# filippo-orru/path-tracer-rust

Measured on AMD Instinct MI355X. Metric: ray_bounces_per_sec, higher is better.
Workload: dtype f32

## Files before the change

### path-tracer-rust_amd/csrc/pt_kernels.hip

```cpp
#include <cstdio>
#include <cstdlib>
#include <string>

#include "pt_kernels.h"
#ifdef PT_TU_TILE
#include "pt_tile.h"
#endif

namespace pt {

#ifdef PT_TU_TILE
typedef TileParams MegaParams;
#define k_mega k_tile_mega
#define k_mega_cand k_tile_mega_cand
#else
typedef FrameParams MegaParams;
#endif
#if defined(PT_TU_FLAT) || defined(PT_TU_TILE)
#define PT_TU_PART 1
#endif

void set_error(const std::string &m);

extern __shared__ uint4 dyn_lds[];

constexpr uint32_t kCandDeferFlush = 64;

__device__ __forceinline__ uint32_t rfl(uint32_t v) { return (uint32_t)__builtin_amdgcn_readfirstlane((int)v); }
__device__ __forceinline__ uint32_t lane_prefix(uint64_t mask) {
    return __builtin_amdgcn_mbcnt_hi((uint32_t)(mask >> 32), __builtin_amdgcn_mbcnt_lo((uint32_t)mask, 0u));
}

struct StreamSlice {
    char *base;
    uint32_t off_tp, off_od1;
};
__device__ __forceinline__ StreamSlice slice_of(const RayQueue &q, uint32_t b, uint32_t cap) {
    StreamSlice s;
    s.base = q.buf + (size_t)b * cap * kRayBytes;
    s.off_tp = cap * 16u;
    s.off_od1 = cap * 32u;
    return s;
}
__device__ __forceinline__ float4 ld_od0(const StreamSlice &q, uint32_t i) { return *reinterpret_cast<const float4 *>(q.base + i * 16u); }
__device__ __forceinline__ float4 ld_tp(const StreamSlice &q, uint32_t i) { return *reinterpret_cast<const float4 *>(q.base + (i * 16u + q.off_tp)); }
__device__ __forceinline__ float2 ld_od1(const StreamSlice &q, uint32_t i) { return *reinterpret_cast<const float2 *>(q.base + (i * 8u + q.off_od1)); }
__device__ __forceinline__ void store_ray(const StreamSlice &q, uint32_t slot, vec3 o, vec3 d, vec3 thr, uint32_t word) {
    *reinterpret_cast<float4 *>(q.base + slot * 16u) = make_float4(o.x, o.y, o.z, d.x);
    *reinterpret_cast<float2 *>(q.base + (slot * 8u + q.off_od1)) = make_float2(d.y, d.z);
    *reinterpret_cast<float4 *>(q.base + (slot * 16u + q.off_tp)) = make_float4(thr.x, thr.y, thr.z, __uint_as_float(word));
}
__device__ __forceinline__ void load_ray_slice(const StreamSlice &q, uint32_t i, vec3 &o, vec3 &d, vec3 &thr, uint32_t &word) {
    const float4 a = ld_od0(q, i);
    const float4 tp = ld_tp(q, i);
    const float2 c = ld_od1(q, i);
    o = mk(a.x, a.y, a.z);
    d = mk(a.w, c.x, c.y);
    thr = mk(tp.x, tp.y, tp.z);
    word = __float_as_uint(tp.w);
}
__device__ __forceinline__ void load_ray_slice(const StreamSlice &q, uint32_t i, RayRows &ray, f32x4 &tp) {
    const f32x2 *a = reinterpret_cast<const f32x2 *>(q.base + i * 16u);
    ray.p0 = a[0];
    ray.p1 = a[1];
    tp = *reinterpret_cast<const f32x4 *>(q.base + (i * 16u + q.off_tp));
    ray.p2 = *reinterpret_cast<const f32x2 *>(q.base + (i * 8u + q.off_od1));
}

#ifndef PT_TU_PART
template <bool PROBE>
__global__ __launch_bounds__(kBlock) void k_generate(FrameParams F, RayQueue q, uint32_t *__restrict__ cnt0,
                                                     uint32_t cap, uint32_t s0, uint32_t s_here, uint32_t m) {
    const uint32_t b = blockIdx.x, tid = threadIdx.x;
    const StreamSlice qs = slice_of(q, b, cap);
    const uint32_t mb = stream_pixel_count(F.npix, F.n_streams, b);
    const uint32_t n = mb * s_here;
    for (uint32_t g = tid; g < n; g += kBlock) {
        const uint32_t pl = stream_pixel(F.n_streams, b, g % mb);
        const uint32_t s = s0 + g / mb;
        const PathRay r = primary_ray<PROBE>(F, global_pixel(F, pl), s);
        store_ray(qs, g, r.o, r.d, r.thr, pack_word(g % mb, g / mb, PROBE ? F.depth0 : 0u, 1u));
    }
    if (tid == 0) cnt0[b] = n;
}

constexpr uint32_t kParkCap = 128;
__host__ __device__ inline size_t bvh_park_offset(const DevScene &S, uint32_t block) {
    return (bvh_lds_bytes(S, block) + 15) & ~(size_t)15;
}
__host__ __device__ inline size_t bvh_park_bytes(uint32_t block) { return (size_t)(block / 64u) * kParkCap * 36u; }

template <bool BVH>
__global__ __launch_bounds__(BVH ? kBlockBvh : kBlock, BVH ? 5 : 1) void k_intersect(DevScene S, RayQueue q, float2 *__restrict__ hit,
                                                      const uint32_t *__restrict__ cnt, uint32_t cap,
                                                      unsigned long long *__restrict__ blk_rays) {
    const uint32_t b = blockIdx.x, tid = threadIdx.x;
    const uint32_t n = cnt[b];
    const size_t base = (size_t)b * cap;
    const StreamSlice qs = slice_of(q, b, cap);
    if (!BVH) {
        for (uint32_t i = tid; i < n; i += blockDim.x) {
            const float4 a = ld_od0(qs, i);
            const float2 c = ld_od1(qs, i);
            const HitRec h = intersect_scene_dev<false>(S, mk(a.x, a.y, a.z), mk(a.w, c.x, c.y), dyn_lds);
            hit[base + i] = make_float2(h.t, __int_as_float(h.id));
        }
    } else {
        if (n != 0u) stage_bvh(S, dyn_lds);
        char *park = reinterpret_cast<char *>(dyn_lds) + bvh_park_offset(S, blockDim.x) + (size_t)(tid >> 6) * kParkCap * 36u;
        float4 *const pa = reinterpret_cast<float4 *>(park), *const pb = pa + kParkCap;
        uint32_t *const pi = reinterpret_cast<uint32_t *>(pb + kParkCap);
        const uint32_t lane = tid & 63u;
        uint32_t n_park = 0;
        auto walk = [&](uint32_t e, bool valid) {
            if (valid) {
                const float4 a = pa[e], bq = pb[e];
                const uint32_t idx = pi[e];
                const vec3 o = mk(a.x, a.y, a.z), d = mk(a.w, bq.x, bq.y);
                float best_t = bq.z;
                int32_t best_id = __float_as_int(bq.w);
                if (walk_deferred(S, o, d, dyn_lds, best_t, best_id)) {
                    const HitRec h = scan_scene<true, true>(S, o, d, dyn_lds);
                    best_t = h.t;
                    best_id = h.id;
                }
                hit[base + idx] = make_float2(best_t, __int_as_float(best_id));
            }
        };
        for (uint32_t j0 = 0; j0 < n; j0 += blockDim.x) {
            const uint32_t i = j0 + tid;
            bool want = false;
            vec3 o = mk(0, 0, 0), d = o;
            HitRec h;
            h.t = 0.0f;
            h.id = -1;
            if (i < n) {
                const float4 a = ld_od0(qs, i);
                const float2 c = ld_od1(qs, i);
                o = mk(a.x, a.y, a.z);
                d = mk(a.w, c.x, c.y);
                h = intersect_scene_dev<true, true>(S, o, d, dyn_lds, &want);
                if (!want) hit[base + i] = make_float2(h.t, __int_as_float(h.id));
            }
            const uint64_t mw = __builtin_amdgcn_ballot_w64(want);
            if (mw != 0ull) {
                if (want) {
                    const uint32_t e = n_park + lane_prefix(mw);
                    pa[e] = make_float4(o.x, o.y, o.z, d.x);
                    pb[e] = make_float4(d.y, d.z, h.t, __int_as_float(h.id));
                    pi[e] = i;
                }
                n_park += (uint32_t)__builtin_popcountll(mw);
            }
            if (n_park >= 64u) {
                n_park -= 64u;
                walk(n_park + lane, true);
            }
        }
        if (n_park != 0u) walk(lane, lane < n_park);
    }
    if (tid == 0) blk_rays[b] += n;
}

#endif

template <bool STAGED>
__global__ __launch_bounds__(kBlock, PT_ISECT_WAVES) void k_intersect_cand(DevScene S, RayQueue q, float2 *__restrict__ hit,
                                                              const uint32_t *__restrict__ cnt, uint32_t cap,
                                                              unsigned long long *__restrict__ blk_rays) {
    const uint32_t b = blockIdx.x, tid = threadIdx.x, lane = tid & 63u;
    const uint32_t n = cnt[b];
    if (n == 0u) return;
    CandLds cand;
    {
        char *wbase = reinterpret_cast<char *>(dyn_lds) + (size_t)(tid >> 6) * kCandWaveBytes;
        cand.ray_a = reinterpret_cast<float4 *>(wbase);
        cand.keys = reinterpret_cast<unsigned long long *>(wbase + 128u * 16u);
        cand.ray_b = reinterpret_cast<float2 *>(wbase + 128u * 24u);
        cand.queue = reinterpret_cast<uint16_t *>(wbase + 128u * 32u);
        char *sbase = reinterpret_cast<char *>(dyn_lds) + intersect_cand_lds_bytes();
        cand.staged = reinterpret_cast<const CandPairRec *>(sbase);
        cand.surf = S.surf;
        if (STAGED) {
            const uint4 *src = reinterpret_cast<const uint4 *>(S.cand_pairs);
            uint4 *dst = reinterpret_cast<uint4 *>(sbase);
            const uint32_t n_rows = S.n_cand_pairs * (uint32_t)(sizeof(CandPairRec) / 16u);
            for (uint32_t k = tid; k < n_rows; k += kBlock) dst[k] = src[k];
            __syncthreads();
        }
    }
    const StreamSlice qin = slice_of(q, b, cap);
    float2 *const hit_b = hit + (size_t)b * cap;
    CandRing ring;
    ring.head = 0u;
    ring.count = 0u;
    const uint32_t n_chunks = (n + kBlock - 1u) / kBlock;
    bool prev_valid = false;
#if PT_ISECT_PREFETCH
    float4 na = make_float4(0.0f, 0.0f, 0.0f, 0.0f);
    float2 nc = make_float2(0.0f, 0.0f);
    if (tid < n) {
        na = ld_od0(qin, tid);
        nc = ld_od1(qin, tid);
    }
#endif
    for (uint32_t it = 0; it <= n_chunks; ++it) {
        const uint32_t par = it & 1u;
        const uint32_t i = it * kBlock + tid;
        const bool cur_valid = it < n_chunks && i < n;
        const uint32_t pending = ring.count;
        bool ran_batch = false;
        if (it < n_chunks) {
            vec3 o = mk(0.0f, 0.0f, 0.0f), d = o;
#if PT_ISECT_PREFETCH
            if (cur_valid) {
                o = mk(na.x, na.y, na.z);
                d = mk(na.w, nc.x, nc.y);
            }
// ... 173 lines not shown
    float4 *const dbuf = reinterpret_cast<float4 *>(reinterpret_cast<char *>(dyn_lds) + pass_lds_defer_offset(m)) +
                         (size_t)(tid >> 6) * (3u * kDeferCap);
    uint32_t n_defer = 0;
    StreamSlice qout{};
    uint32_t *tail_p = nullptr;
    auto append = [&](const ShadeOut &so, uint32_t word) {
        const uint64_t m1 = __builtin_amdgcn_ballot_w64(so.n_rays >= 1);
        const uint64_t m2 = __builtin_amdgcn_ballot_w64(so.n_rays == 2);
        const uint32_t c1 = (uint32_t)__builtin_popcountll(m1), c2 = (uint32_t)__builtin_popcountll(m2);
        if ((c1 + c2) == 0u) return;
        uint32_t wbase = 0;
        if ((tid & 63u) == 0u) wbase = atomicAdd(tail_p, c1 + c2);
        wbase = (uint32_t)__builtin_amdgcn_readfirstlane((int)wbase);
        if (so.n_rays >= 1) {
            const uint32_t slot = wbase + lane_prefix(m1);
            if (slot < cap)
                store_ray(qout, slot, so.x, so.d0, so.thr0,
                          pack_word(word_pix(word), word_sample(word), meta_depth(so.meta0), meta_branch(so.meta0)));
            else
                overflow = true;
        }
        if (so.n_rays == 2) {
            const uint32_t slot = wbase + c1 + lane_prefix(m2);
            if (slot < cap)
                store_ray(qout, slot, so.x, so.d1, so.thr1,
                          pack_word(word_pix(word), word_sample(word), meta_depth(so.meta1), meta_branch(so.meta1)));
            else
                overflow = true;
        }
    };
    auto shade_deferred = [&](uint32_t e, bool valid) {
        ShadeOut so;
        so.n_rays = 0;
        so.emits = false;
        uint32_t word = 0;
        if (valid) {
            const float4 a = dbuf[e], bq = dbuf[kDeferCap + e], cq = dbuf[2u * kDeferCap + e];
            PathRay in;
            in.o = mk(a.x, a.y, a.z);
            in.d = mk(a.w, bq.x, bq.y);
            in.thr = mk(bq.z, bq.w, cq.x);
            word = __float_as_uint(cq.y);
            HitRec h;
            h.t = cq.z;
            h.id = __float_as_int(cq.w);
            in.pix = lds_pix[word_pix(word)];
            in.meta = pack_meta(s0 + word_sample(word), word_depth(word), word_branch(word));
            shade_hit<kShadeRefractOnly>(S, P, in, h, so);
            if (so.emits) add_radiance_lds(lds_acc, m, word_pix(word), so.contrib);
        }
        append(so, word);
    };
    for (uint32_t depth = 0; depth < (uint32_t)kMaxDepth && n != 0u; ++depth) {
        const StreamSlice qin = slice_of((depth & 1u) ? q1 : q0, b, cap);
        qout = slice_of((depth & 1u) ? q0 : q1, b, cap);
        __syncthreads();
        if (tid == 0) s_tail_p[(depth + 1u) & 1u] = 0u;
        tail_p = s_tail_p + (depth & 1u);
        total += n;
        for (uint32_t j0 = 0; j0 < n; j0 += kBlock) {
            const uint32_t i = j0 + tid;
            PathRay in;
            uint32_t word = 0;
            if (i < n) {
                if (depth == 0u) {
                    const uint32_t pj = i % mb, sj = i / mb;
                    in = primary_ray<PROBE>(F, lds_pix[pj], s0 + sj);
                    word = pack_word(pj, sj, PROBE ? F.depth0 : 0u, 1u);
                } else {
                    const float4 a = ld_od0(qin, i);
                    const float4 tp = ld_tp(qin, i);
                    const float2 c = ld_od1(qin, i);
                    in.o = mk(a.x, a.y, a.z);
                    in.d = mk(a.w, c.x, c.y);
                    in.thr = mk(tp.x, tp.y, tp.z);
                    word = __float_as_uint(tp.w);
                }
            }
            ShadeOut so;
            so.n_rays = 0;
            so.emits = false;
            so.deferred = false;
            HitRec h;
            h.t = 0.0f;
            h.id = -1;
            if (i < n) {
                h = intersect_scene_dev<false>(S, in.o, in.d, nullptr);
                if (h.id >= 0) {
                    in.pix = lds_pix[word_pix(word)];
                    in.meta = pack_meta(s0 + word_sample(word), word_depth(word), word_branch(word));
                    shade_hit<DEFER ? kShadeDeferRefract : kShadeAll>(S, P, in, h, so);
                    if (so.emits) add_radiance_lds(lds_acc, m, word_pix(word), so.contrib);
                }
            }
            append(so, word);
            const uint64_t md = DEFER ? __builtin_amdgcn_ballot_w64(so.deferred) : 0ull;
            if (DEFER && md != 0ull) {
                if (so.deferred) {
                    const uint32_t e = n_defer + lane_prefix(md);
                    dbuf[e] = make_float4(in.o.x, in.o.y, in.o.z, in.d.x);
                    dbuf[kDeferCap + e] = make_float4(in.d.y, in.d.z, in.thr.x, in.thr.y);
                    dbuf[2u * kDeferCap + e] = make_float4(in.thr.z, __uint_as_float(word), h.t, __int_as_float(h.id));
                }
                n_defer = rfl(n_defer + (uint32_t)__builtin_popcountll(md));
            }
            if (DEFER && n_defer >= 64u) {
                n_defer -= 64u;
                shade_deferred(n_defer + (tid & 63u), true);
            }
        }
        if (DEFER && n_defer != 0u) {
            shade_deferred(tid & 63u, (tid & 63u) < n_defer);
            n_defer = 0u;
        }
        __syncthreads();
        const uint32_t tail = *tail_p;
        n = tail < cap ? tail : cap;
    }
    if (overflow) atomicOr(flags, 1u);
    __syncthreads();
    if (tid == 0) blk_rays[b] += total;
    const size_t plane = (size_t)F.n_streams * m;
    for (uint32_t k = tid; k < 3u * mb; k += kBlock) {
        const uint32_t c = k / mb, p = k - c * mb;
        const unsigned long long v = lds_acc[c * m + p];
        if (v) acc[(size_t)c * plane + (size_t)b * m + p] += v;
    }
}

#endif
constexpr uint32_t kCandParkCap = kWaveParkCap;

template <bool STAGED, bool DEFER, bool BVH, bool PROBE, bool NLDS = false>
__global__ __launch_bounds__(kBlock, BVH ? PT_CAND_BVH_WAVES : PT_CAND_WAVES) void k_pass_cand(DevScene S, FrameParams F, RayQueue q0, RayQueue q1, uint32_t cap,
                                                         uint32_t s0, uint32_t s_here, uint32_t m,
                                                         unsigned long long *__restrict__ acc,
                                                         unsigned long long *__restrict__ blk_rays,
                                                         uint32_t *__restrict__ flags) {
    unsigned long long *lds_acc = reinterpret_cast<unsigned long long *>(dyn_lds);
    uint32_t *s_tail_p = reinterpret_cast<uint32_t *>(lds_acc + pass_acc_slots(m));
    const uint32_t b = blockIdx.x, tid = threadIdx.x, lane = tid & 63u;
    const uint32_t mb = stream_pixel_count(F.npix, F.n_streams, b);
    if (mb == 0u) return;
#ifdef PT_PHASE_STATS
    unsigned long long ph_t0, ph_r0;
    phase_begin(&ph_t0, &ph_r0);
#endif
    for (uint32_t k = tid; k < 3u * m; k += kBlock) lds_acc[k] = 0ull;
    if (tid == 0) s_tail_p[0] = s_tail_p[1] = 0u;
    if (tid == 0) {
        float *cw = reinterpret_cast<float *>(s_tail_p + 4);
        cw[0] = F.lens_x, cw[1] = F.lens_y, cw[2] = F.lens_z, cw[3] = F.cam_px, cw[4] = F.cam_py, cw[5] = F.cam_pz;
        cw[6] = F.su_x, cw[7] = F.su_y, cw[8] = F.su_z, cw[9] = F.sv_x, cw[10] = F.sv_y, cw[11] = F.sv_z;
        s_tail_p[16] = F.width, s_tail_p[17] = F.height;
    }
    uint32_t *lds_pix = s_tail_p + kPassTailWords;
    uint32_t *lds_px = lds_pix + m, *lds_py = lds_px + m;
    for (uint32_t j = tid; j < mb; j += kBlock) {
        const uint32_t pix = global_pixel(F, stream_pixel(F.n_streams, b, j));
        lds_pix[j] = pix;
        lds_px[j] = pix % F.width;
        lds_py[j] = F.height - 1u - pix / F.width;
    }
    const uint32_t wv = (uint32_t)__builtin_amdgcn_readfirstlane((int)(tid >> 6));
    const uint32_t cap_w = cap >> 2;
    const uint32_t n0 = mb * s_here;
    const uint32_t n_chunks = (n0 + 63u) >> 6;
    const uint32_t my_chunks = (n_chunks + 3u - wv) >> 2;
    const uint32_t quarter = (((n_chunks + 3u) >> 2) << 6) < n0 ? (((n_chunks + 3u) >> 2) << 6) : n0;
    const uint32_t base0 = wv << 6;
    uint32_t gen_left = 0u;
    if (my_chunks != 0u) {
        const uint32_t last = wv + ((my_chunks - 1u) << 2);
        gen_left = ((my_chunks - 1u) << 6) + (n0 - (last << 6) < 64u ? n0 - (last << 6) : 64u);
    }
#if PT_SAMPLE_MAJOR
    const uint32_t step_q = 256u / s_here, step_r = 256u % s_here;
    uint32_t gen_pj = (base0 + lane) / s_here, gen_sj = (base0 + lane) % s_here;
#else
    const uint32_t step_q = 256u / mb, step_r = 256u % mb;
    uint32_t gen_pj = (base0 + lane) % mb, gen_sj = (base0 + lane) / mb;
#endif
    CandLds cand;
    const SurfRec *surf_lds = nullptr;
    uint32_t surf_head = 0u;
    {
        char *cbase = reinterpret_cast<char *>(dyn_lds) + pass_lds_cand_offset(m, DEFER);
        char *wbase = cbase + (size_t)(tid >> 6) * kCandWaveBytes;
        cand.ray_a = reinterpret_cast<float4 *>(wbase);
        cand.keys = reinterpret_cast<unsigned long long *>(wbase + 128u * 16u);
        cand.ray_b = reinterpret_cast<float2 *>(wbase + 128u * 24u);
        cand.queue = reinterpret_cast<uint16_t *>(wbase + 128u * 32u);
        char *sbase = cbase + pass_lds_cand_bytes() + (BVH ? pass_cand_bvh_bytes(S) : 0u);
        cand.staged = reinterpret_cast<const CandPairRec *>(sbase);
        cand.surf = S.surf;
        if (STAGED) {
            const uint4 *src = reinterpret_cast<const uint4 *>(S.cand_pairs);
            uint4 *dst = reinterpret_cast<uint4 *>(sbase);
            const uint32_t n_rows = S.n_cand_pairs * (uint32_t)(sizeof(CandPairRec) / 16u);
            for (uint32_t k = tid; k < n_rows; k += kBlock) dst[k] = src[k];
            if (!BVH || S.surf_staged) {
                const uint4 *src2 = reinterpret_cast<const uint4 *>(S.surf);
                uint4 *dst2 = dst + n_rows;
                const uint32_t n_rows2 = (S.n_objs + S.n_tris) * (uint32_t)(sizeof(SurfRec) / 16u);
                for (uint32_t k = tid; k < n_rows2; k += kBlock) dst2[k] = src2[k];
                cand.surf = reinterpret_cast<const SurfRec *>(dst2);
            } else if (S.surf_head != 0u) {
                const uint4 *src2 = reinterpret_cast<const uint4 *>(S.surf);
                uint4 *dst2 = dst + n_rows;
                const uint32_t n_rows2 = S.surf_head * (uint32_t)(sizeof(SurfRec) / 16u);
                for (uint32_t k = tid; k < n_rows2; k += kBlock) dst2[k] = src2[k];
                surf_lds = reinterpret_cast<const SurfRec *>(dst2);
                surf_head = S.surf_head;
            }
        }
    }
    char *const walk_lds = (reinterpret_cast<char *>(dyn_lds) + pass_lds_cand_offset(m, DEFER) + pass_lds_cand_bytes());
    unsigned long long *p_key = nullptr;
    unsigned long long *walk_keys = nullptr;
    WalkQueue wq{};
    const WalkNode *const nodes_lds = reinterpret_cast<const WalkNode *>(walk_lds + pass_cand_nodes_offset(S));
    if (BVH && NLDS) {
        const uint4 *src = reinterpret_cast<const uint4 *>(walk_nodes(S));
        uint4 *dst = reinterpret_cast<uint4 *>(walk_lds + pass_cand_nodes_offset(S));
        for (uint32_t k = tid; k < walk_node_count(S) * (uint32_t)(sizeof(WalkNode) / 16u); k += kBlock) dst[k] = src[k];
    }
    if (BVH) {
        walk_keys = reinterpret_cast<unsigned long long *>(walk_lds + pass_cand_queues_bytes(S) + (size_t)(tid >> 6) * kCandWalkKeyBytes);
        char *qb = walk_lds + (size_t)(tid >> 6) * pass_cand_queue_bytes(S);
        wq.redo = reinterpret_cast<uint32_t *>(qb);
        wq.ent = reinterpret_cast<uint2 *>(qb + kWalkQueueHeader);
        wq.cap = (uint32_t)((pass_cand_queue_bytes(S) - kWalkQueueHeader) / 8u);
        if (S.walk_queue_cap >= 128u && S.walk_queue_cap < wq.cap) wq.cap = S.walk_queue_cap;
    }
    ShadeParams P;
    P.idx_begin = F.idx_begin;
    P.npix = F.npix;
    P.n_streams = F.n_streams;
    {
        uint32_t k_lo = F.seed_lo, k_hi = F.seed_hi;
        asm volatile("" : "+s"(k_lo), "+s"(k_hi));
        P.seed_lo = k_lo;
        P.seed_hi = k_hi;
    }
    P.debug = F.debug;
    P.s0 = s0;
    P.chunk_pixels = F.chunk_pixels;
    P.chunk_first = F.chunk_first;
    P.chunk_step = F.chunk_step;
    P.k_begin = F.k_begin;
    bool overflow = false;
    unsigned long long total = 0ull;
    const uint32_t room = cap_w < kWaveStackMax ? cap_w : kWaveStackMax;
    const bool room_for_all = 4u * quarter + 3u <= room;
    StreamSlice qs;
    qs.base = q0.buf + (size_t)(b * 4u + wv) * cap_w * kRayBytes;
    qs.off_tp = room * 16u;
    qs.off_od1 = room * 32u;
    StreamSlice qpark{};
    if (BVH || DEFER) {
        qpark.base = q1.buf + (size_t)(b * 4u + wv) * kWaveParkBytes;
        qpark.off_tp = kCandParkCap * 16u;
        qpark.off_od1 = kCandParkCap * 32u;
        p_key = reinterpret_cast<unsigned long long *>(qpark.base + kCandParkCap * kRayBytes);
    }
    if (!room_for_all && room < 512u) {
        if (tid == 0) atomicOr(flags, 2u);
        return;
    }
    uint32_t top = 0u;
    auto append = [&](const ShadeOut &so, uint32_t word) {
        PT_PHASE(kPhAppend);
        const uint64_t m1 = __builtin_amdgcn_ballot_w64(so.n_rays >= 1);
        const uint64_t m2 = __builtin_amdgcn_ballot_w64(so.n_rays == 2);
        const uint32_t c1 = (uint32_t)__builtin_popcountll(m1), c2 = (uint32_t)__builtin_popcountll(m2);
        if ((c1 + c2) == 0u) return;
        const uint32_t wbase = top;
        if (wbase + c1 + c2 > room) {
            overflow = true;
            return;
        }
        top = rfl(top + c1 + c2);
        if (so.n_rays >= 1)
            store_ray(qs, wbase + lane_prefix(m1), so.x, so.d0, so.thr0,
                      pack_word(word_pix(word), word_sample(word), meta_depth(so.meta0), meta_branch(so.meta0)));
        if (so.n_rays == 2) {
            PT_PHASE(kPhAppend2);
            store_ray(qs, wbase + c1 + lane_prefix(m2), so.x, so.d1, so.thr1,
                      pack_word(word_pix(word), word_sample(word), meta_depth(so.meta1), meta_branch(so.meta1)));
        }
    };
    uint32_t n_defer = 0;
    auto shade_deferred = [&](uint32_t e, bool valid) {
        ShadeOut so;
        so.n_rays = 0;
        so.emits = false;
        uint32_t word = 0;
        PT_PHASE(kPhDefer);
        __builtin_amdgcn_fence(__ATOMIC_RELEASE, "wavefront");
        __builtin_amdgcn_fence(__ATOMIC_ACQUIRE, "wavefront");
        if (valid) {
            PathRay in;
            load_ray_slice(qpark, e, in.o, in.d, in.thr, word);
            const unsigned long long hk = p_key[e];
            in.pix = lds_pix[word_pix(word)];
            in.meta = pack_meta(s0 + word_sample(word), word_depth(word), word_branch(word));
            const Surface sf = fetch_surface_rank(cand.surf, in.o, in.d, __uint_as_float((uint32_t)(hk >> 32)), (uint32_t)hk);
            shade_surface<kShadeRefractOnly>(P, in, sf, so);
            PT_PHASE(kPhEmit);
            if (so.emits) add_radiance_lds(lds_acc, m, word_pix(word), so.contrib);
        }
        append(so, word);
    };
    uint32_t n_park = 0;
    auto walk_batch = [&](uint32_t e, bool valid) {
        ShadeOut so;
        so.n_rays = 0;
        so.emits = false;
        uint32_t word = 0;
        PT_PHASE(kPhLoad);
        __builtin_amdgcn_fence(__ATOMIC_RELEASE, "wavefront");
        __builtin_amdgcn_fence(__ATOMIC_ACQUIRE, "wavefront");
        if (valid) {
            PathRay in;
            load_ray_slice(qpark, e, in.o, in.d, in.thr, word);
            unsigned long long key;
            if constexpr (NLDS)
                key = walk_deferred_keys(S, nodes_lds, in.o, in.d, wq, p_key[e], walk_keys);
            else
                key = walk_deferred_keys(S, walk_nodes(S), in.o, in.d, wq, p_key[e], walk_keys);
            const uint32_t rank = (uint32_t)key;
            if (rank != 0xffffffffu) {
                in.pix = lds_pix[word_pix(word)];
                in.meta = pack_meta(s0 + word_sample(word), word_depth(word), word_branch(word));
                PT_PHASE(kPhSurface);
                const Surface sf = fetch_surface_rank(cand.surf, in.o, in.d, __uint_as_float((uint32_t)(key >> 32)), rank, surf_lds, surf_head);
                shade_surface<kShadeAll>(P, in, sf, so);
                PT_PHASE(kPhEmit);
                if (so.emits) add_radiance_lds(lds_acc, m, word_pix(word), so.contrib);
            }
        }
        append(so, word);
    };
    CandRing ring;
    ring.head = 0u;
    ring.count = 0u;
    PT_PHASE(kPhBarrier);
    __syncthreads();
    PT_PHASE(kPhOther);
    uint32_t par = 0u;
    bool pending = false;
    vec3 prev_thr = mk(0.0f, 0.0f, 0.0f);
    uint32_t prev_word = 0;
    bool prev_valid = false;
    for (;;) {
        const uint32_t phi = 2u * top + 4u * (n_park + n_defer + (pending ? 64u : 0u));
        const bool may_start = gen_left != 0u && (room_for_all || phi + 256u <= room);
        uint32_t src = 0u, cnt = 0u;
        if (top >= 64u) {
            src = 1u;
            cnt = 64u;
        } else if (may_start) {
            src = 2u;
            cnt = gen_left < 64u ? gen_left : 64u;
        } else if (top != 0u) {
            src = 1u;
            cnt = top;
        }
        src = rfl(src);
        cnt = rfl(cnt);
        const bool idle = src == 0u && !pending;
        if (idle && n_defer == 0u && n_park == 0u) break;
        const bool cur_valid = lane < cnt;
        vec3 cur_thr = mk(0.0f, 0.0f, 0.0f);
        uint32_t word = 0;
        const uint32_t pend_entries = ring.count;
        bool ran_batch = false;
        if (src != 0u) {
            RayRows ray;
            if (src == 2u) {
                PT_PHASE(kPhPrimary);
                PathRay in;
                in.o = in.d = in.thr = mk(0.0f, 0.0f, 0.0f);
                if (cur_valid) {
                    const uint32_t pj = gen_pj, sj = gen_sj;
                    FrameParams Fl;
                    {
                        const float4 c0 = *reinterpret_cast<const float4 *>(s_tail_p + 4), c1 = *reinterpret_cast<const float4 *>(s_tail_p + 8),
                                     c2 = *reinterpret_cast<const float4 *>(s_tail_p + 12);
                        Fl.lens_x = c0.x, Fl.lens_y = c0.y, Fl.lens_z = c0.z, Fl.cam_px = c0.w, Fl.cam_py = c1.x, Fl.cam_pz = c1.y;
                        Fl.su_x = c1.z, Fl.su_y = c1.w, Fl.su_z = c2.x, Fl.sv_x = c2.y, Fl.sv_y = c2.z, Fl.sv_z = c2.w;
                        Fl.width = s_tail_p[16], Fl.height = s_tail_p[17];
                        Fl.seed_lo = P.seed_lo, Fl.seed_hi = P.seed_hi;
                    }
                    in = PROBE ? primary_ray<PROBE>(F, lds_pix[pj], s0 + sj) : primary_ray_at(Fl, lds_pix[pj], lds_px[pj], lds_py[pj], s0 + sj);
                    word = pack_word(pj, sj, PROBE ? F.depth0 : 0u, 1u);
                }
#if PT_SAMPLE_MAJOR
                gen_sj += step_r;
                gen_pj += step_q;
                if (gen_sj >= s_here) {
                    gen_sj -= s_here;
                    gen_pj += 1u;
                }
#else
                gen_pj += step_r;
                gen_sj += step_q;
                if (gen_pj >= mb) {
                    gen_pj -= mb;
                    gen_sj += 1u;
                }
#endif
                gen_left = rfl(gen_left - cnt);
                ray = ray_rows(in.o, in.d);
                cur_thr = in.thr;
            } else {
                PT_PHASE(kPhLoad);
                __builtin_amdgcn_fence(__ATOMIC_RELEASE, "wavefront");
                __builtin_amdgcn_fence(__ATOMIC_ACQUIRE, "wavefront");
                top = rfl(top - cnt);
                f32x4 tp;
                load_ray_slice(qs, top + (lane < cnt - 1u ? lane : cnt - 1u), ray, tp);
                cur_thr = mk(tp[0], tp[1], tp[2]);
                word = __float_as_uint(tp[3]);
            }
            total += cnt;
            const uint32_t slot = (par << 6) | lane;
            cand.ray_a[slot] = make_float4(ray.p0[0], ray.p0[1], ray.p1[0], ray.p1[1]);
            cand.ray_b[slot] = make_float2(ray.p2[0], ray.p2[1]);
            float bound;
            PT_PHASE(kPhSpheres);
            const unsigned long long key0 = cand_spheres(S, ray, &bound);
            cand.keys[slot] = cur_valid ? key0 : kKeyMiss;
            const uint32_t before = ring.head;
            cand_filter_and_drain<STAGED>(S, cand, ring, lane, par, __builtin_amdgcn_uicmp(lane, cnt, 36 ), ray, bound);
            ran_batch = ring.head != before;
        }
        if (pending) {
            PT_PHASE(kPhFinish);
            if (pend_entries != 0u && !ran_batch) cand_batch<STAGED>(S, cand, ring, lane, ring.count);
            PT_PHASE(kPhFinish);
            ShadeOut so;
            so.n_rays = 0;
            so.emits = false;
            so.deferred = false;
            float hit_t = 0.0f;
            uint32_t hit_rank = 0xffffffffu;
            PathRay pr;
            pr.o = pr.d = pr.thr = mk(0.0f, 0.0f, 0.0f);
            bool park = false;
            unsigned long long park_key = 0ull;
            if (prev_valid) {
                const uint32_t slot = ((par ^ 1u) << 6) | lane;
                const unsigned long long key = load_key(&cand.keys[slot]);
                const uint32_t rank = (uint32_t)key;
                if (BVH) {
                    const float4 ra = cand.ray_a[slot];
                    const float2 rb = cand.ray_b[slot];
                    pr.o = mk(ra.x, ra.y, ra.z);
                    pr.d = mk(ra.w, rb.x, rb.y);
                    park = bvh_wants(S, pr.o, pr.d, __uint_as_float((uint32_t)(key >> 32)));
                    park_key = key;
                }
                if (rank != 0xffffffffu && !park) {
                    hit_t = __uint_as_float((uint32_t)(key >> 32));
                    hit_rank = rank;
                    if (!BVH) {
                        const float4 ra = cand.ray_a[slot];
                        const float2 rb = cand.ray_b[slot];
                        pr.o = mk(ra.x, ra.y, ra.z);
                        pr.d = mk(ra.w, rb.x, rb.y);
                    }
                    pr.thr = prev_thr;
                    pr.pix = lds_pix[word_pix(prev_word)];
                    pr.meta = pack_meta(s0 + word_sample(prev_word), word_depth(prev_word), word_branch(prev_word));
                    PT_PHASE(kPhSurface);
                    const Surface sf = fetch_surface_rank(cand.surf, pr.o, pr.d, hit_t, rank, surf_lds, surf_head);
                    PT_PHASE_PIN(sf.n.x);
                    PT_PHASE_PIN(sf.n.y);
                    PT_PHASE_PIN(sf.n.z);
                    PT_PHASE_PIN(sf.x.x);
                    shade_surface<DEFER ? kShadeDeferRefract : kShadeAll>(P, pr, sf, so);
                    PT_PHASE(kPhEmit);
                    if (so.emits) {
                        PT_PHASE(kPhEmitAdd);
                        add_radiance_lds(lds_acc, m, word_pix(prev_word), so.contrib);
                    }
                }
            }
            append(so, prev_word);
            if (BVH) {
                const uint64_t mw = __builtin_amdgcn_ballot_w64(park);
                PT_WSTAT(S, 7, __builtin_popcountll(__builtin_amdgcn_ballot_w64(prev_valid)));
                PT_WSTAT(S, 8, __builtin_popcountll(mw));
                PT_WSTAT(S, 9, 1);
                if (mw != 0ull) {
                    if (park) {
                        const uint32_t e = n_park + lane_prefix(mw);
                        store_ray(qpark, e, pr.o, pr.d, prev_thr, prev_word);
                        p_key[e] = park_key;
                    }
                    n_park = rfl(n_park + (uint32_t)__builtin_popcountll(mw));
                }
            }
            PT_PHASE(kPhDefer);
            const uint64_t md = DEFER ? __builtin_amdgcn_ballot_w64(so.deferred) : 0ull;
            if (DEFER && md != 0ull) {
                if (so.deferred) {
                    const uint32_t e = n_defer + lane_prefix(md);
                    store_ray(qpark, e, pr.o, pr.d, pr.thr, prev_word);
                    p_key[e] = ((unsigned long long)__float_as_uint(hit_t) << 32) | hit_rank;
                }
                n_defer = rfl(n_defer + (uint32_t)__builtin_popcountll(md));
            }
        }
        while (BVH && (n_park >= 64u || (idle && n_park != 0u))) {
            const uint32_t c = n_park < 64u ? n_park : 64u;
            n_park = rfl(n_park - c);
            walk_batch(n_park + lane, lane < c);
        }
        if (DEFER && (n_defer >= kCandDeferFlush || (idle && n_defer != 0u))) {
            const uint32_t c = n_defer < 64u ? n_defer : 64u;
            n_defer = rfl(n_defer - c);
            shade_deferred(n_defer + lane, lane < c);
        }
        PT_PHASE(kPhOther);
        prev_thr = cur_thr;
        prev_word = word;
        prev_valid = cur_valid;
        pending = src != 0u;
        par = rfl(par ^ 1u);
    }
    if (overflow) atomicOr(flags, 1u);
    if (lane == 0u) atomicAdd(reinterpret_cast<unsigned long long *>(s_tail_p), total);
    PT_PHASE(kPhBarrier);
    __syncthreads();
    PT_PHASE(kPhOther);
    if (tid == 0) blk_rays[b] += *reinterpret_cast<unsigned long long *>(s_tail_p);
    const size_t plane = (size_t)F.n_streams * m;
    for (uint32_t k = tid; k < 3u * mb; k += kBlock) {
        const uint32_t c = k / mb, p = k - c * mb;
        const unsigned long long v = lds_acc[c * m + p];
        if (v) acc[(size_t)c * plane + (size_t)b * m + p] += v;
    }
#ifdef PT_PHASE_STATS
    phase_end(S.phase_stats, ph_t0, ph_r0);
#endif
}

#ifndef PT_TU_PART
constexpr uint32_t kPassParkCap = 128;
__host__ __device__ inline size_t pass_bvh_stack_offset(uint32_t m) { return pass_lds_defer_offset(m); }
__host__ __device__ inline size_t pass_bvh_park_offset(const DevScene &S, uint32_t m) {
    return (pass_bvh_stack_offset(m) + (size_t)kBvhStack * kBlock * ((S.bvh_in_lds & 2u) ? sizeof(uint16_t) : sizeof(uint32_t)) + 15) &
           ~(size_t)15;
}
__host__ __device__ inline size_t pass_bvh_leaf_offset(const DevScene &S, uint32_t m) {
    return (pass_bvh_park_offset(S, m) + (size_t)(kBlock / 64u) * kPassParkCap * 12u + 15) & ~(size_t)15;
}
__host__ __device__ inline size_t pass_bvh_lds_bytes(const DevScene &S, uint32_t m) {
    return pass_bvh_leaf_offset(S, m) + (size_t)(kBlock / 64u) * (64u * 8u + kLeafListCap * 4u);
}

template <bool PROBE>
__global__ __launch_bounds__(kBlock, 4) void k_pass_bvh(DevScene S, FrameParams F, RayQueue q0, RayQueue q1, uint32_t cap,
                                                        uint32_t s0, uint32_t s_here, uint32_t m,
                                                        unsigned long long *__restrict__ acc,
                                                        unsigned long long *__restrict__ blk_rays,
                                                        uint32_t *__restrict__ flags) {
    unsigned long long *lds_acc = reinterpret_cast<unsigned long long *>(dyn_lds);
    uint32_t *s_tail_p = reinterpret_cast<uint32_t *>(lds_acc + pass_acc_slots(m));
    const uint32_t b = blockIdx.x, tid = threadIdx.x, lane = tid & 63u;
    const uint32_t mb = stream_pixel_count(F.npix, F.n_streams, b);
    if (mb == 0u) return;
    for (uint32_t k = tid; k < 3u * m; k += kBlock) lds_acc[k] = 0ull;
    if (tid == 0) s_tail_p[0] = s_tail_p[1] = 0u;
    uint32_t *lds_pix = s_tail_p + kPassTailWords;
    for (uint32_t j = tid; j < mb; j += kBlock) lds_pix[j] = global_pixel(F, stream_pixel(F.n_streams, b, j));
    uint4 *const stacks = reinterpret_cast<uint4 *>(reinterpret_cast<char *>(dyn_lds) + pass_bvh_stack_offset(m));
    char *park = reinterpret_cast<char *>(dyn_lds) + pass_bvh_park_offset(S, m) + (size_t)(tid >> 6) * kPassParkCap * 12u;
    uint32_t *const p_idx = reinterpret_cast<uint32_t *>(park);
    float *const p_t = reinterpret_cast<float *>(p_idx + kPassParkCap);
    int32_t *const p_id = reinterpret_cast<int32_t *>(p_t + kPassParkCap);
    LeafLds leaves;
    {
        char *lbase = reinterpret_cast<char *>(dyn_lds) + pass_bvh_leaf_offset(S, m) + (size_t)(tid >> 6) * (64u * 8u + kLeafListCap * 4u);
        leaves.keys = reinterpret_cast<unsigned long long *>(lbase);
        leaves.list = reinterpret_cast<uint32_t *>(lbase + 64u * 8u);
    }
    ShadeParams P;
    P.idx_begin = F.idx_begin;
    P.npix = F.npix;
    P.n_streams = F.n_streams;
    P.seed_lo = F.seed_lo;
    P.seed_hi = F.seed_hi;
    P.debug = F.debug;
    P.s0 = s0;
    P.chunk_pixels = F.chunk_pixels;
    P.chunk_first = F.chunk_first;
    P.chunk_step = F.chunk_step;
    P.k_begin = F.k_begin;
    bool overflow = false;
    unsigned long long total = 0ull;
    uint32_t n = mb * s_here;
    __syncthreads();
    for (uint32_t g = tid; g < n; g += kBlock) {
        const uint32_t pj = g % mb, sj = g / mb;
        const PathRay r = primary_ray<PROBE>(F, lds_pix[pj], s0 + sj);
        store_ray(slice_of(q0, b, cap), g, r.o, r.d, r.thr, pack_word(pj, sj, PROBE ? F.depth0 : 0u, 1u));
    }
    uint32_t n_park = 0;
    StreamSlice qin{}, qout{};
    uint32_t *tail_p = nullptr;
    auto append = [&](const ShadeOut &so, uint32_t word) {
        const uint64_t m1 = __builtin_amdgcn_ballot_w64(so.n_rays >= 1);
        const uint64_t m2 = __builtin_amdgcn_ballot_w64(so.n_rays == 2);
        const uint32_t c1 = (uint32_t)__builtin_popcountll(m1), c2 = (uint32_t)__builtin_popcountll(m2);
        if ((c1 + c2) == 0u) return;
        uint32_t wbase = 0;
        if (lane == 0u) wbase = atomicAdd(tail_p, c1 + c2);
        wbase = (uint32_t)__builtin_amdgcn_readfirstlane((int)wbase);
        if (so.n_rays >= 1) {
            const uint32_t slot = wbase + lane_prefix(m1);
            if (slot < cap)
                store_ray(qout, slot, so.x, so.d0, so.thr0,
                          pack_word(word_pix(word), word_sample(word), meta_depth(so.meta0), meta_branch(so.meta0)));
            else
                overflow = true;
        }
        if (so.n_rays == 2) {
            const uint32_t slot = wbase + c1 + lane_prefix(m2);
            if (slot < cap)
                store_ray(qout, slot, so.x, so.d1, so.thr1,
                          pack_word(word_pix(word), word_sample(word), meta_depth(so.meta1), meta_branch(so.meta1)));
            else
                overflow = true;
        }
    };
    auto load_ray = [&](uint32_t i, PathRay &in, uint32_t &word) {
        const float4 a = ld_od0(qin, i);
        const float4 tp = ld_tp(qin, i);
        const float2 c = ld_od1(qin, i);
        in.o = mk(a.x, a.y, a.z);
        in.d = mk(a.w, c.x, c.y);
        in.thr = mk(tp.x, tp.y, tp.z);
        word = __float_as_uint(tp.w);
    };
    auto shade_and_append = [&](bool valid, PathRay &in, uint32_t word, HitRec h) {
        ShadeOut so;
        so.n_rays = 0;
        so.emits = false;
        if (valid && h.id >= 0) {
            in.pix = lds_pix[word_pix(word)];
            in.meta = pack_meta(s0 + word_sample(word), word_depth(word), word_branch(word));
            shade_hit(S, P, in, h, so);
            if (so.emits) add_radiance_lds(lds_acc, m, word_pix(word), so.contrib);
        }
        append(so, word);
    };
    auto walk_batch = [&](uint32_t e, bool valid) {
        PathRay in;
        uint32_t word = 0;
        HitRec h;
        h.t = 0.0f;
        h.id = -1;
        if (valid) {
            load_ray(p_idx[e], in, word);
            h.t = p_t[e];
            h.id = p_id[e];
            if (walk_deferred(S, in.o, in.d, stacks, h.t, h.id, &leaves))
                h = scan_scene<true, true>(S, in.o, in.d, stacks);
        }
        shade_and_append(valid, in, word, h);
    };
    for (uint32_t depth = 0; depth < (uint32_t)kMaxDepth && n != 0u; ++depth) {
        qin = slice_of((depth & 1u) ? q1 : q0, b, cap);
        qout = slice_of((depth & 1u) ? q0 : q1, b, cap);
        __syncthreads();
        if (tid == 0) s_tail_p[(depth + 1u) & 1u] = 0u;
        tail_p = s_tail_p + (depth & 1u);
        total += n;
// ... 923 lines not shown
```

### path-tracer-rust_amd/csrc/pt_layout.h

```cpp
#pragma once

#include <cstdio>
#include <string>

#include "pt_device.h"

namespace pt {

#ifndef PT_CAND_WAVES
#define PT_CAND_WAVES 5
#endif
#ifndef PT_ISECT_WAVES
#define PT_ISECT_WAVES 4
#endif
#ifndef PT_CAND_BVH_WAVES
#define PT_CAND_BVH_WAVES 4
#endif

constexpr uint32_t kDeferCap = 128;
constexpr uint32_t kPassTailWords = 20;
PT_HDC uint32_t pass_acc_slots(uint32_t m) { return (3u * m + 1u) & ~1u; }
PT_HDC size_t pass_lds_defer_offset(uint32_t m) {
    return ((size_t)pass_acc_slots(m) * sizeof(unsigned long long) + kPassTailWords * 4u + (size_t)3 * m * sizeof(uint32_t) + 15) & ~(size_t)15;
}
static_assert(pass_acc_slots(1) == 4u && pass_acc_slots(2) == 6u && (pass_acc_slots(7) * 8u) % 16u == 0u, "tails are 16-byte aligned");

PT_HDC size_t pass_lds_cand_offset(uint32_t m, bool ) { return pass_lds_defer_offset(m); }
constexpr size_t kCandWaveBytes = 128u * 16u + 128u * 8u + 128u * 8u + kCandQueueCap * 2u;
PT_HDC size_t pass_lds_cand_bytes() { return (size_t)(kBlock / 64u) * kCandWaveBytes; }
static_assert(kCandWaveBytes % 16u == 0u, "per-wave areas stay 16-byte aligned");

PT_HDC size_t intersect_cand_lds_bytes() { return (size_t)(kBlock / 64u) * kCandWaveBytes; }

#ifndef PT_WALK_QUEUE_BYTES
#define PT_WALK_QUEUE_BYTES 3584
#endif
constexpr uint32_t kWalkQueueBytes = PT_WALK_QUEUE_BYTES;
constexpr uint32_t kWalkQueueBytesStaged = 2048;
PT_HDI size_t pass_cand_queue_bytes(const DevScene &S) {
    const size_t again = (size_t)S.bvh_stack * 64u * ((S.bvh_in_lds & 2u) ? 2u : 4u) + kLeafListCap * 4u;
    const size_t q = (S.bvh_in_lds & 4u) ? kWalkQueueBytesStaged : kWalkQueueBytes;
    return kWalkQueueHeader + (((again > q ? again : q) + 15) & ~(size_t)15);
}
PT_HDI size_t pass_cand_queues_bytes(const DevScene &S) { return (size_t)(kBlock / 64u) * pass_cand_queue_bytes(S); }
constexpr size_t kCandWalkKeyBytes = 64u * 8u;
PT_HDI size_t pass_cand_nodes_offset(const DevScene &S) {
    return pass_cand_queues_bytes(S) + (size_t)(kBlock / 64u) * kCandWalkKeyBytes;
}
PT_HDI size_t pass_cand_bvh_bytes(const DevScene &S) {
    return pass_cand_nodes_offset(S) + ((S.bvh_in_lds & 4u) ? (size_t)walk_node_count(S) * sizeof(WalkNode) : 0u);
}
static_assert(kCandWalkKeyBytes % 16u == 0u && sizeof(WalkNode) % 16u == 0u, "per-wave areas stay 16-byte aligned");

PT_HDC size_t mega_spare_bytes(uint32_t depth) { return (size_t)depth * kBlock * 16u; }
constexpr size_t kMegaOwnerBytes = kBlock * sizeof(uint32_t);
constexpr size_t kMegaLdsBudget = 40u * 1024u;

enum PassKernel : uint32_t {
    kPassPlain = 0,
    kPassDefer = 1,
    kPassCand = 2,
    kPassCandBvh = 3,
};

struct LdsLayout {
    uint32_t pass;
    uint32_t m;
    bool staged;
    bool defer;
    bool nodes_lds;
    uint32_t bvh_in_lds;
    uint32_t surf_staged;
    uint32_t surf_head;
    size_t pass_lds;
    size_t pass_pad;
    bool isect_staged;
    size_t isect_lds;
    bool mega_cand;
    uint32_t mega_depth;
    uint32_t mega_spare_off;
    uint32_t mega_surf_off;
    size_t mega_lds;
};

inline LdsLayout lds_layout(const DevScene &S, uint32_t m, size_t lds_pad) {
    LdsLayout L{};
    L.m = m;
    const bool bvh = S.n_bvh_nodes != 0u;
    const size_t rec_cand = (size_t)S.n_cand_pairs * sizeof(CandPairRec);
    const size_t rec_surf = (size_t)(S.n_objs + S.n_tris) * sizeof(SurfRec);
    L.bvh_in_lds = S.bvh_in_lds;
    if (S.cand_scan) {
        const size_t budget = 160u * 1024u / (bvh ? PT_CAND_BVH_WAVES : PT_CAND_WAVES) - (bvh ? 0u : 512u);
        DevScene S2 = S;
        S2.bvh_in_lds &= ~1u;
        L.defer = !bvh && S.glass_defer_ok;
        if (bvh && S.nodes_in_lds_ok) {
            DevScene S3 = S2;
            S3.bvh_in_lds |= 4u;
            L.nodes_lds = pass_lds_cand_offset(m, false) + pass_lds_cand_bytes() + pass_cand_bvh_bytes(S3) + rec_cand <= budget;
            if (L.nodes_lds) S2 = S3;
        }
        const size_t walk = bvh ? pass_cand_bvh_bytes(S2) : 0u;
        const size_t before = pass_lds_cand_offset(m, L.defer) + pass_lds_cand_bytes() + walk;
        L.surf_staged = before + rec_cand + rec_surf <= budget ? 1u : 0u;
        L.staged = bvh ? (L.surf_staged || before + rec_cand <= budget + 8u * 1024u) : L.surf_staged != 0u;
        if (bvh && L.staged && !L.surf_staged && before + rec_cand < budget) {
            const size_t fit = (budget - before - rec_cand) / sizeof(SurfRec);
            const size_t n_ranks = (size_t)S.n_objs + S.n_tris;
            L.surf_head = (uint32_t)(fit < n_ranks ? fit : n_ranks);
        }
        L.pass = bvh ? kPassCandBvh : kPassCand;
        L.bvh_in_lds = S2.bvh_in_lds;
        L.pass_lds = before + (L.staged ? rec_cand + (L.surf_staged ? rec_surf : (size_t)L.surf_head * sizeof(SurfRec)) : 0u);
        L.pass_pad = lds_pad;
    } else {
        const size_t lds_plain = pass_lds_defer_offset(m);
        const size_t lds_defer = lds_plain + (size_t)(kBlock / 64u) * 3u * kDeferCap * 16u;
        L.defer = lds_defer <= 32u * 1024u;
        L.pass = L.defer ? kPassDefer : kPassPlain;
        L.pass_lds = L.defer ? lds_defer : lds_plain;
    }
    L.isect_staged = intersect_cand_lds_bytes() + rec_cand <= 160u * 1024u / PT_ISECT_WAVES;
    L.isect_lds = intersect_cand_lds_bytes() + (L.isect_staged ? rec_cand : 0u);
    const size_t rec = (rec_cand + 15) & ~(size_t)15;
    DevScene S4 = S;
    S4.bvh_in_lds &= ~5u;
    const size_t mwalk = bvh ? pass_cand_queues_bytes(S4) + (size_t)(kBlock / 64u) * kCandWalkKeyBytes : 0u;
    const size_t base = intersect_cand_lds_bytes() + rec + mwalk;
    L.mega_cand = S.cand_scan && base + mega_spare_bytes(2) + kMegaOwnerBytes <= kMegaLdsBudget;
    if (L.mega_cand) {
        L.mega_depth = base + mega_spare_bytes(4) + kMegaOwnerBytes <= kMegaLdsBudget ? 4u : 2u;
        L.mega_spare_off = (uint32_t)base;
        const size_t after = base + mega_spare_bytes(L.mega_depth) + kMegaOwnerBytes;
        L.mega_surf_off = after + rec_surf <= kMegaLdsBudget ? (uint32_t)after : 0u;
        L.mega_lds = after + (L.mega_surf_off ? rec_surf : 0u);
    } else {
        L.mega_lds = bvh_lds_bytes(S, kBlock);
    }
    return L;
}

inline std::string lds_layout_line(const LdsLayout &L, int which) {
    char buf[256];
    if (which == 0 && L.pass == kPassCand)
        snprintf(buf, sizeof buf, "k_pass_cand: %zu bytes of LDS per workgroup (+ %zu of padding), m = %u, staged %d, defer %d",
                 L.pass_lds, L.pass_pad, L.m, (int)L.staged, (int)L.defer);
    else if (which == 0 && L.pass == kPassCandBvh)
        snprintf(buf, sizeof buf,
                 "k_pass_cand<BVH>: %zu bytes of LDS per workgroup (+ %zu of padding), m = %u, staged %d, nodes_lds %d, surf_staged %u, surf_head %u",
                 L.pass_lds, L.pass_pad, L.m, (int)L.staged, (int)L.nodes_lds, L.surf_staged, L.surf_head);
    else if (which == 0)
        snprintf(buf, sizeof buf, "k_pass: %zu bytes of LDS per workgroup (+ 0 of padding), m = %u, defer %d", L.pass_lds, L.m, (int)L.defer);
    else if (which == 1)
        snprintf(buf, sizeof buf, "k_intersect_cand: %zu bytes of LDS per workgroup (+ 0 of padding), staged %d", L.isect_lds,
                 (int)L.isect_staged);
    else if (L.mega_cand)
        snprintf(buf, sizeof buf, "k_mega_cand: %zu bytes of LDS per workgroup (+ 0 of padding), depth %u, spare_off %u, surf_off %u",
                 L.mega_lds, L.mega_depth, L.mega_spare_off, L.mega_surf_off);
    else
        snprintf(buf, sizeof buf, "k_mega: %zu bytes of LDS per workgroup (+ 0 of padding)", L.mega_lds);
    return buf;
}

}
```

Baseline: 58.56 billion.

## Park waiting ray throughput/word in LDS to cut registers in non-BVH candidate pass

For the non-BVH candidate pass, each thread's pending ray throughput and packed word are kept in a per-thread LDS row instead of live registers across the batch. The row is read back and refilled after the candidate batch, and sample-index advancing is deferred until then. The LDS tail is shrunk, a wait area is added to the layout, and target waves per CU rise from 5 to 6 with a tighter LDS budget. This trades extra LDS traffic and less LDS for staging for lower register pressure and higher occupancy.

```diff
diff --git a/path-tracer-rust_amd/csrc/pt_kernels.hip b/path-tracer-rust_amd/csrc/pt_kernels.hip
--- a/path-tracer-rust_amd/csrc/pt_kernels.hip
+++ b/path-tracer-rust_amd/csrc/pt_kernels.hip
@@ -64,6 +64,12 @@
     ray.p0 = a[0];
     ray.p1 = a[1];
     tp = *reinterpret_cast<const f32x4 *>(q.base + (i * 16u + q.off_tp));
+    ray.p2 = *reinterpret_cast<const f32x2 *>(q.base + (i * 8u + q.off_od1));
+}
+__device__ __forceinline__ void load_ray_slice(const StreamSlice &q, uint32_t i, RayRows &ray) {
+    const f32x2 *a = reinterpret_cast<const f32x2 *>(q.base + i * 16u);
+    ray.p0 = a[0];
+    ray.p1 = a[1];
     ray.p2 = *reinterpret_cast<const f32x2 *>(q.base + (i * 8u + q.off_od1));
 }
 
@@ -543,7 +549,7 @@
         float *cw = reinterpret_cast<float *>(s_tail_p + 4);
         cw[0] = F.lens_x, cw[1] = F.lens_y, cw[2] = F.lens_z, cw[3] = F.cam_px, cw[4] = F.cam_py, cw[5] = F.cam_pz;
         cw[6] = F.su_x, cw[7] = F.su_y, cw[8] = F.su_z, cw[9] = F.sv_x, cw[10] = F.sv_y, cw[11] = F.sv_z;
-        s_tail_p[16] = F.width, s_tail_p[17] = F.height;
+        s_tail_p[2] = F.width, s_tail_p[3] = F.height;
     }
     uint32_t *lds_pix = s_tail_p + kPassTailWords;
     uint32_t *lds_px = lds_pix + m, *lds_py = lds_px + m;
@@ -582,7 +588,7 @@
         cand.keys = reinterpret_cast<unsigned long long *>(wbase + 128u * 16u);
         cand.ray_b = reinterpret_cast<float2 *>(wbase + 128u * 24u);
         cand.queue = reinterpret_cast<uint16_t *>(wbase + 128u * 32u);
-        char *sbase = cbase + pass_lds_cand_bytes() + (BVH ? pass_cand_bvh_bytes(S) : 0u);
+        char *sbase = cbase + pass_lds_cand_bytes() + pass_lds_wait_bytes(BVH) + (BVH ? pass_cand_bvh_bytes(S) : 0u);
         cand.staged = reinterpret_cast<const CandPairRec *>(sbase);
         cand.surf = S.surf;
         if (STAGED) {
@@ -741,6 +747,24 @@
     PT_PHASE(kPhOther);
     uint32_t par = 0u;
     bool pending = false;
+    float4 *const wait_row = reinterpret_cast<float4 *>(reinterpret_cast<char *>(dyn_lds) + pass_lds_wait_offset(m)) + tid;
+    auto gen_advance = [&]() {
+#if PT_SAMPLE_MAJOR
+        gen_sj += step_r;
+        gen_pj += step_q;
+        if (gen_sj >= s_here) {
+            gen_sj -= s_here;
+            gen_pj += 1u;
+        }
+#else
+        gen_pj += step_r;
+        gen_sj += step_q;
+        if (gen_pj >= mb) {
+            gen_pj -= mb;
+            gen_sj += 1u;
+        }
+#endif
+    };
     vec3 prev_thr = mk(0.0f, 0.0f, 0.0f);
     uint32_t prev_word = 0;
     bool prev_valid = false;
@@ -781,39 +805,29 @@
                                      c2 = *reinterpret_cast<const float4 *>(s_tail_p + 12);
                         Fl.lens_x = c0.x, Fl.lens_y = c0.y, Fl.lens_z = c0.z, Fl.cam_px = c0.w, Fl.cam_py = c1.x, Fl.cam_pz = c1.y;
                         Fl.su_x = c1.z, Fl.su_y = c1.w, Fl.su_z = c2.x, Fl.sv_x = c2.y, Fl.sv_y = c2.z, Fl.sv_z = c2.w;
-                        Fl.width = s_tail_p[16], Fl.height = s_tail_p[17];
+                        Fl.width = s_tail_p[2], Fl.height = s_tail_p[3];
                         Fl.seed_lo = P.seed_lo, Fl.seed_hi = P.seed_hi;
                     }
                     in = PROBE ? primary_ray<PROBE>(F, lds_pix[pj], s0 + sj) : primary_ray_at(Fl, lds_pix[pj], lds_px[pj], lds_py[pj], s0 + sj);
-                    word = pack_word(pj, sj, PROBE ? F.depth0 : 0u, 1u);
-                }
-#if PT_SAMPLE_MAJOR
-                gen_sj += step_r;
-                gen_pj += step_q;
-                if (gen_sj >= s_here) {
-                    gen_sj -= s_here;
-                    gen_pj += 1u;
-                }
-#else
-                gen_pj += step_r;
-                gen_sj += step_q;
-                if (gen_pj >= mb) {
-                    gen_pj -= mb;
-                    gen_sj += 1u;
-                }
-#endif
+                    if constexpr (BVH) word = pack_word(pj, sj, PROBE ? F.depth0 : 0u, 1u);
+                }
+                if constexpr (BVH) gen_advance();
                 gen_left = rfl(gen_left - cnt);
                 ray = ray_rows(in.o, in.d);
-                cur_thr = in.thr;
+                if constexpr (BVH) cur_thr = in.thr;
             } else {
                 PT_PHASE(kPhLoad);
                 __builtin_amdgcn_fence(__ATOMIC_RELEASE, "wavefront");
                 __builtin_amdgcn_fence(__ATOMIC_ACQUIRE, "wavefront");
                 top = rfl(top - cnt);
-                f32x4 tp;
-                load_ray_slice(qs, top + (lane < cnt - 1u ? lane : cnt - 1u), ray, tp);
-                cur_thr = mk(tp[0], tp[1], tp[2]);
-                word = __float_as_uint(tp[3]);
+                if constexpr (BVH) {
+                    f32x4 tp;
+                    load_ray_slice(qs, top + (lane < cnt - 1u ? lane : cnt - 1u), ray, tp);
+                    cur_thr = mk(tp[0], tp[1], tp[2]);
+                    word = __float_as_uint(tp[3]);
+                } else {
+                    load_ray_slice(qs, top + (lane < cnt - 1u ? lane : cnt - 1u), ray);
+                }
             }
             total += cnt;
             const uint32_t slot = (par << 6) | lane;
@@ -830,6 +844,19 @@
         if (pending) {
             PT_PHASE(kPhFinish);
             if (pend_entries != 0u && !ran_batch) cand_batch<STAGED>(S, cand, ring, lane, ring.count);
+        }
+        if constexpr (!BVH) {
+            const float4 w = *wait_row;
+            prev_thr = mk(w.x, w.y, w.z);
+            prev_word = __float_as_uint(w.w);
+            if (src == 1u) {
+                *wait_row = ld_tp(qs, top + (lane < cnt - 1u ? lane : cnt - 1u));
+            } else if (src == 2u) {
+                *wait_row = make_float4(1.0f, 1.0f, 1.0f, __uint_as_float(pack_word(gen_pj, gen_sj, PROBE ? F.depth0 : 0u, 1u)));
+                gen_advance();
+            }
+        }
+        if (pending) {
             PT_PHASE(kPhFinish);
             ShadeOut so;
             so.n_rays = 0;
@@ -916,8 +943,10 @@
             shade_deferred(n_defer + lane, lane < c);
         }
         PT_PHASE(kPhOther);
-        prev_thr = cur_thr;
-        prev_word = word;
+        if constexpr (BVH) {
+            prev_thr = cur_thr;
+            prev_word = word;
+        }
         prev_valid = cur_valid;
         pending = src != 0u;
         par = rfl(par ^ 1u);
diff --git a/path-tracer-rust_amd/csrc/pt_layout.h b/path-tracer-rust_amd/csrc/pt_layout.h
--- a/path-tracer-rust_amd/csrc/pt_layout.h
+++ b/path-tracer-rust_amd/csrc/pt_layout.h
@@ -8,7 +8,7 @@
 namespace pt {
 
 #ifndef PT_CAND_WAVES
-#define PT_CAND_WAVES 5
+#define PT_CAND_WAVES 6
 #endif
 #ifndef PT_ISECT_WAVES
 #define PT_ISECT_WAVES 4
@@ -18,7 +18,7 @@
 #endif
 
 constexpr uint32_t kDeferCap = 128;
-constexpr uint32_t kPassTailWords = 20;
+constexpr uint32_t kPassTailWords = 16;
 PT_HDC uint32_t pass_acc_slots(uint32_t m) { return (3u * m + 1u) & ~1u; }
 PT_HDC size_t pass_lds_defer_offset(uint32_t m) {
     return ((size_t)pass_acc_slots(m) * sizeof(unsigned long long) + kPassTailWords * 4u + (size_t)3 * m * sizeof(uint32_t) + 15) & ~(size_t)15;
@@ -29,6 +29,10 @@
 constexpr size_t kCandWaveBytes = 128u * 16u + 128u * 8u + 128u * 8u + kCandQueueCap * 2u;
 PT_HDC size_t pass_lds_cand_bytes() { return (size_t)(kBlock / 64u) * kCandWaveBytes; }
 static_assert(kCandWaveBytes % 16u == 0u, "per-wave areas stay 16-byte aligned");
+
+PT_HDC size_t pass_lds_wait_bytes(bool bvh) { return bvh ? 0u : (size_t)kBlock * 16u; }
+PT_HDC size_t pass_lds_wait_offset(uint32_t m) { return pass_lds_cand_offset(m, false) + pass_lds_cand_bytes(); }
+static_assert((pass_lds_wait_offset(1) % 16u) == 0u && (pass_lds_wait_offset(7) % 16u) == 0u, "rows are read and written as b128");
 
 PT_HDC size_t intersect_cand_lds_bytes() { return (size_t)(kBlock / 64u) * kCandWaveBytes; }
 
@@ -83,6 +87,10 @@
     size_t mega_lds;
 };
 
+PT_HDC size_t pass_cand_lds_budget(bool bvh) {
+    return bvh ? 160u * 1024u / PT_CAND_BVH_WAVES : (PT_CAND_WAVES == 6 ? 26880u : 160u * 1024u / PT_CAND_WAVES - 512u);
+}
+
 inline LdsLayout lds_layout(const DevScene &S, uint32_t m, size_t lds_pad) {
     LdsLayout L{};
     L.m = m;
@@ -91,7 +99,7 @@
     const size_t rec_surf = (size_t)(S.n_objs + S.n_tris) * sizeof(SurfRec);
     L.bvh_in_lds = S.bvh_in_lds;
     if (S.cand_scan) {
-        const size_t budget = 160u * 1024u / (bvh ? PT_CAND_BVH_WAVES : PT_CAND_WAVES) - (bvh ? 0u : 512u);
+        const size_t budget = pass_cand_lds_budget(bvh);
         DevScene S2 = S;
         S2.bvh_in_lds &= ~1u;
         L.defer = !bvh && S.glass_defer_ok;
@@ -102,7 +110,7 @@
             if (L.nodes_lds) S2 = S3;
         }
         const size_t walk = bvh ? pass_cand_bvh_bytes(S2) : 0u;
-        const size_t before = pass_lds_cand_offset(m, L.defer) + pass_lds_cand_bytes() + walk;
+        const size_t before = pass_lds_cand_offset(m, L.defer) + pass_lds_cand_bytes() + pass_lds_wait_bytes(bvh) + walk;
         L.surf_staged = before + rec_cand + rec_surf <= budget ? 1u : 0u;
         L.staged = bvh ? (L.surf_staged || before + rec_cand <= budget + 8u * 1024u) : L.surf_staged != 0u;
         if (bvh && L.staged && !L.surf_staged && before + rec_cand < budget) {
```

Result: faster. 60.64 billion (median of 6 runs) (+3.5%).
